# cruzryan/OpenDOG

Hardware: NVIDIA B200
Metric: env-steps/sec (device-timed) at 1/2/4/8 B200 vs ref mj_step on host cores (higher is better)
Workload: dtype f32

## Files before the change

### opendog_b200/csrc/odg_core.cuh

```cuda
#pragma once

#include <stdint.h>
#include <math.h>
#include <string.h>

#ifdef ODG_HOST_EMU
#define ODG_DEV inline
#define ODG_NOINLINE inline
#define ODG_RESTRICT
struct float4 { float x, y, z, w; };
float odg_emu_shfl_xor(float v, int m);
double odg_emu_shfl_xor_d(double v, int m);
static inline float odg_rsqrt(float x) { return 1.0f / sqrtf(x); }
static inline float odg_fmul_rn(float a, float b) { volatile float r = a * b; return r; }
static inline float odg_fadd_rn(float a, float b) { volatile float r = a + b; return r; }
static inline float odg_fsub_rn(float a, float b) { volatile float r = a - b; return r; }
static inline float odg_fdiv_rn(float a, float b) { volatile float r = a / b; return r; }
static inline float odg_fdiv_fast(float a, float b) { return a / b; }
static inline float odg_fma_rn(float a, float b, float c) { return fmaf(a, b, c); }
#ifdef ODG_EMU_STATS
void odg_emu_stat(int it, float rel_step, float alpha, int ls_passes, int nc_leg, float d10);
#endif
#define ODG_UNROLL
#define ODG_NO_UNROLL
// ... 93 lines not shown
  const float* mean;
  float* actions;
  float* cost;
};

struct StepArgs {
  const float* action;
  float* obs;
  float* reward;
  unsigned char* terminated; unsigned char* truncated;
  int mode;
  int want_info;
  float* x_position; float* y_position; float* distance; float* paw_forces; float* patterns_matches;
  float* lin_vel_reward; float* reward_ctrl; float* terminal_obs; unsigned char* paws_in_ground;
  int* gait_reward; float* qacc; int* ncon; float* fn_sum; int* solver_iters; int* ls_evals;
  float* reward_raw;
  float* cfrc_ext;
  float* task_terms;
};

struct V3 { float x, y, z; };
ODG_DEV V3 mk3(float x, float y, float z) { V3 r; r.x = x; r.y = y; r.z = z; return r; }
ODG_DEV V3 operator+(V3 a, V3 b) { return mk3(a.x + b.x, a.y + b.y, a.z + b.z); }
ODG_DEV V3 operator-(V3 a, V3 b) { return mk3(a.x - b.x, a.y - b.y, a.z - b.z); }
ODG_DEV V3 operator*(float s, V3 a) { return mk3(s * a.x, s * a.y, s * a.z); }
ODG_DEV V3 operator-(V3 a) { return mk3(-a.x, -a.y, -a.z); }
ODG_DEV float dot3(float ax, float ay, float az, float bx, float by, float bz) {
  return odg_fma_rn(az, bz, odg_fma_rn(ay, by, odg_fmul_rn(ax, bx)));
}
ODG_DEV float dot(V3 a, V3 b) { return dot3(a.x, a.y, a.z, b.x, b.y, b.z); }
ODG_DEV float cross1(float a, float b, float c, float d) { return odg_fma_rn(a, b, -odg_fmul_rn(c, d)); }
ODG_DEV V3 cross(V3 a, V3 b) { return mk3(cross1(a.y, b.z, a.z, b.y), cross1(a.z, b.x, a.x, b.z), cross1(a.x, b.y, a.y, b.x)); }
ODG_DEV float dot_acc(float acc, V3 a, V3 b) { return odg_fma_rn(a.z, b.z, odg_fma_rn(a.y, b.y, odg_fma_rn(a.x, b.x, acc))); }
ODG_DEV float cross1_acc(float acc, float a, float b, float c, float d) { return odg_fma_rn(a, b, odg_fma_rn(-c, d, acc)); }
ODG_DEV V3 cross_acc(V3 acc, V3 a, V3 b) {
  return mk3(cross1_acc(acc.x, a.y, b.z, a.z, b.y), cross1_acc(acc.y, a.z, b.x, a.x, b.z), cross1_acc(acc.z, a.x, b.y, a.y, b.x));
}
ODG_DEV float comp(V3 a, int i) { return i == 0 ? a.x : (i == 1 ? a.y : a.z); }

ODG_DEV float4 mk4(V3 v, float w) { float4 r; r.x = v.x; r.y = v.y; r.z = v.z; r.w = w; return r; }
ODG_DEV V3 xyz(float4 q) { return mk3(q.x, q.y, q.z); }
#ifdef ODG_HOST_EMU
static inline float odg_int_bits(int i) { float f; memcpy(&f, &i, 4); return f; }
static inline int odg_float_bits(float f) { int i; memcpy(&i, &f, 4); return i; }
#else
#define odg_int_bits __int_as_float
#define odg_float_bits __float_as_int
#endif

struct M3 { float m[9]; };
ODG_DEV V3 mul(const M3& R, V3 v) {
  return mk3(dot3(R.m[0], R.m[1], R.m[2], v.x, v.y, v.z), dot3(R.m[3], R.m[4], R.m[5], v.x, v.y, v.z),
             dot3(R.m[6], R.m[7], R.m[8], v.x, v.y, v.z));
}
ODG_DEV V3 tmul(const M3& R, V3 v) {
  return mk3(dot3(R.m[0], R.m[3], R.m[6], v.x, v.y, v.z), dot3(R.m[1], R.m[4], R.m[7], v.x, v.y, v.z),
             dot3(R.m[2], R.m[5], R.m[8], v.x, v.y, v.z));
}
ODG_DEV M3 mul(const M3& A, const M3& B) {
  M3 C;
  ODG_UNROLL for (int i = 0; i < 3; i++)
    ODG_UNROLL for (int j = 0; j < 3; j++)
      C.m[i * 3 + j] = A.m[i * 3] * B.m[j] + A.m[i * 3 + 1] * B.m[3 + j] + A.m[i * 3 + 2] * B.m[6 + j];
  return C;
}
ODG_DEV V3 col(const M3& R, int k) { return mk3(R.m[k], R.m[3 + k], R.m[6 + k]); }

struct S3 { float xx, xy, xz, yy, yz, zz; };
ODG_DEV V3 mul(const S3& A, V3 v) {
  return mk3(dot3(A.xx, A.xy, A.xz, v.x, v.y, v.z), dot3(A.xy, A.yy, A.yz, v.x, v.y, v.z),
             dot3(A.xz, A.yz, A.zz, v.x, v.y, v.z));
}
ODG_DEV S3 zero_s3() { S3 s; s.xx = s.xy = s.xz = s.yy = s.yz = s.zz = 0.f; return s; }
ODG_DEV void add_outer(S3& A, V3 a, V3 b) {
  A.xx += a.x * b.x; A.xy += a.x * b.y; A.xz += a.x * b.z; A.yy += a.y * b.y; A.yz += a.y * b.z; A.zz += a.z * b.z;
}
ODG_DEV S3 rotate_sym(const M3& R, const S3& A) {
  V3 c0 = mul(A, mk3(R.m[0], R.m[1], R.m[2]));
  V3 c1 = mul(A, mk3(R.m[3], R.m[4], R.m[5]));
  V3 c2 = mul(A, mk3(R.m[6], R.m[7], R.m[8]));
  V3 r0 = mk3(R.m[0], R.m[1], R.m[2]), r1 = mk3(R.m[3], R.m[4], R.m[5]), r2 = mk3(R.m[6], R.m[7], R.m[8]);
  S3 o;
  o.xx = dot(r0, c0); o.xy = dot(r0, c1); o.xz = dot(r0, c2);
  o.yy = dot(r1, c1); o.yz = dot(r1, c2); o.zz = dot(r2, c2);
  return o;
}

struct SpI { float m; V3 h; S3 I; };
ODG_DEV SpI spi_make(float mass, V3 c, const S3& Iw) {
  SpI s; s.m = mass; s.h = mass * c;
  float cc = dot(c, c);
  s.I.xx = Iw.xx + mass * (cc - c.x * c.x); s.I.yy = Iw.yy + mass * (cc - c.y * c.y); s.I.zz = Iw.zz + mass * (cc - c.z * c.z);
  s.I.xy = Iw.xy - mass * c.x * c.y; s.I.xz = Iw.xz - mass * c.x * c.z; s.I.yz = Iw.yz - mass * c.y * c.z;
  return s;
}
ODG_DEV SpI spi_add(const SpI& a, const SpI& b) {
  SpI s; s.m = a.m + b.m; s.h = a.h + b.h;
  s.I.xx = a.I.xx + b.I.xx; s.I.xy = a.I.xy + b.I.xy; s.I.xz = a.I.xz + b.I.xz;
  s.I.yy = a.I.yy + b.I.yy; s.I.yz = a.I.yz + b.I.yz; s.I.zz = a.I.zz + b.I.zz;
  return s;
}

#ifdef ODG_HOST_EMU
ODG_DEV float grp_xor(float v, int m, unsigned) { return odg_emu_shfl_xor(v, m); }
#else
ODG_DEV float grp_xor(float v, int m, unsigned gmask) { return __shfl_xor_sync(gmask, v, m); }
#endif
#ifdef ODG_HOST_EMU
ODG_DEV double grp_xor_d(double v, int m, unsigned) { return odg_emu_shfl_xor_d(v, m); }
#else
ODG_DEV double grp_xor_d(double v, int m, unsigned gmask) { return __shfl_xor_sync(gmask, v, m); }
#endif
#ifdef ODG_HOST_EMU
ODG_DEV void grp_sync(unsigned) { (void)odg_emu_shfl_xor(0.f, 1); }
#else
ODG_DEV void grp_sync(unsigned gmask) { __syncwarp(gmask); }
#endif
ODG_DEV float grp_sum(float v, unsigned gm) { v += grp_xor(v, 1, gm); v += grp_xor(v, 2, gm); return v; }
ODG_DEV float grp_sum21(float v, unsigned gm) { v += grp_xor(v, 2, gm); v += grp_xor(v, 1, gm); return v; }
constexpr int kRedVals = 28, kRedStride = 36, kRedGroup = 4 * kRedStride;
constexpr int kSupportCells = 24;
ODG_DEV void grp_sum28(float (&v)[kRedVals], float* ODG_RESTRICT s_red, int leg, unsigned gm) {
  grp_sync(gm);
  float4* mine = reinterpret_cast<float4*>(s_red + leg * kRedStride);
  ODG_UNROLL for (int k = 0; k < kRedVals / 4; k++) { float4 t; t.x = v[4 * k]; t.y = v[4 * k + 1]; t.z = v[4 * k + 2]; t.w = v[4 * k + 3]; mine[k] = t; }
  grp_sync(gm);
  float4* res = reinterpret_cast<float4*>(s_red);
  ODG_UNROLL for (int h = 0; h < 2; h++) {
    const int k = 2 * leg + h;
    const float4 a = reinterpret_cast<const float4*>(s_red)[k];
    const float4 b = reinterpret_cast<const float4*>(s_red + kRedStride)[k];
    const float4 c = reinterpret_cast<const float4*>(s_red + 2 * kRedStride)[k];
    const float4 d = reinterpret_cast<const float4*>(s_red + 3 * kRedStride)[k];
    float4 t;
    t.x = ((a.x + b.x) + c.x) + d.x; t.y = ((a.y + b.y) + c.y) + d.y; t.z = ((a.z + b.z) + c.z) + d.z; t.w = ((a.w + b.w) + c.w) + d.w;
    res[k] = t;
  }
  grp_sync(gm);
  ODG_UNROLL for (int k = 0; k < kRedVals / 4; k++) {
    const float4 t = res[k];
    v[4 * k] = t.x; v[4 * k + 1] = t.y; v[4 * k + 2] = t.z; v[4 * k + 3] = t.w;
  }
}
ODG_DEV void grp_sum_max2(float& sum, float& m0, float& m1, float* ODG_RESTRICT s_red, int leg, unsigned gm) {
  grp_sync(gm);
  float4 t; t.x = sum; t.y = m0; t.z = m1; t.w = 0.f;
  *reinterpret_cast<float4*>(s_red + leg * kRedStride) = t;
  grp_sync(gm);
  const float4 a = *reinterpret_cast<const float4*>(s_red), b = *reinterpret_cast<const float4*>(s_red + kRedStride);
  const float4 c = *reinterpret_cast<const float4*>(s_red + 2 * kRedStride), d = *reinterpret_cast<const float4*>(s_red + 3 * kRedStride);
  sum = ((a.x + b.x) + c.x) + d.x;
  m0 = fmaxf(fmaxf(a.y, b.y), fmaxf(c.y, d.y));
  m1 = fmaxf(fmaxf(a.z, b.z), fmaxf(c.z, d.z));
}
ODG_DEV float grp_max(float v, unsigned gm) { v = fmaxf(v, grp_xor(v, 1, gm)); v = fmaxf(v, grp_xor(v, 2, gm)); return v; }
ODG_DEV V3 grp_sum(V3 v, unsigned gm) { return mk3(grp_sum(v.x, gm), grp_sum(v.y, gm), grp_sum(v.z, gm)); }
ODG_DEV float grp_bcast(float v, int src_leg, int leg, unsigned gm) {
  float a = grp_xor(v, 1, gm); float m1 = ((leg ^ src_leg) & 1) ? a : v;
  float b = grp_xor(m1, 2, gm); return ((leg ^ src_leg) & 2) ? b : m1;
}

ODG_DEV void philox4x32(uint32_t k0, uint32_t k1, uint32_t c0, uint32_t c1, uint32_t c2, uint32_t c3, uint32_t out[4]) {
  ODG_UNROLL for (int r = 0; r < 10; r++) {
    uint64_t p0 = (uint64_t)0xD2511F53u * c0, p1 = (uint64_t)0xCD9E8D57u * c2;
    uint32_t n0 = (uint32_t)(p1 >> 32) ^ c1 ^ k0, n1 = (uint32_t)p1;
    uint32_t n2 = (uint32_t)(p0 >> 32) ^ c3 ^ k1, n3 = (uint32_t)p0;
    c0 = n0; c1 = n1; c2 = n2; c3 = n3; k0 += 0x9E3779B9u; k1 += 0xBB67AE85u;
  }
  out[0] = c0; out[1] = c1; out[2] = c2; out[3] = c3;
}
ODG_DEV float u01(uint32_t x) { return (float)(x >> 8) * 5.9604644775390625e-08f; }
constexpr uint32_t kStreamReset = 0x52534554u, kStreamDesvel = 0x44564c00u;

constexpr uint32_t kStreamMppi = 0x4d505049u;
#ifndef ODG_HOST_EMU
ODG_DEV void mppi_sample_row(const float* ODG_RESTRICT mean, float sigma, int n, int A, uint32_t seed_lo, uint32_t seed_hi,
                             uint32_t iteration, uint32_t t, float* ODG_RESTRICT action) {
  for (int blk = 0; blk * 4 < A; blk++) {
    uint32_t r[4];
    philox4x32(seed_lo, seed_hi, (uint32_t)n, iteration, (t << 8) | (uint32_t)blk, kStreamMppi, r);
    for (int pr = 0; pr < 2; pr++) {
      const float u1 = ((float)(r[2 * pr] >> 8) + 1.0f) * 5.9604644775390625e-08f;
      const float u2 = u01(r[2 * pr + 1]);
      const float rad = sqrtf(-2.0f * logf(u1));
      float sn, cs; sincosf(6.283185307179586f * u2, &sn, &cs);
      const float e[2] = { rad * cs, rad * sn };
      for (int q = 0; q < 2; q++) {
        const int a = blk * 4 + pr * 2 + q;
        if (a < A) action[(size_t)n * A + a] = fminf(1.f, fmaxf(-1.f, mean[a] + sigma * e[q]));
      }
    }
  }
}
#endif

ODG_NOINLINE float impedance_pow(float x, float mid, float power) {
  return x <= mid ? powf(x, power) / powf(mid, power - 1.f) : 1.f - powf(1.f - x, power) / powf(1.f - mid, power - 1.f);
}
ODG_DEV float impedance(const float* imp5, float pos_minus_margin) {
  const float d0 = imp5[0], d1 = imp5[1], width = imp5[2], mid = imp5[3], power = imp5[4];
  const bool flat = d0 == d1 || width <= 1e-15f;
  const float x = fminf(fabsf(odg_fdiv_fast(pos_minus_margin, flat ? 1.f : width)), 1.f);
  float y;
  if (power == 2.f) {
    const bool low = x <= mid;
    const float t = low ? x : 1.f - x;
    const float q = odg_fdiv_fast(t * t, low ? mid : 1.f - mid);
    y = low ? q : 1.f - q;
  } else if (power == 1.f) {
    y = x;
  } else {
    y = (x <= 0.f) ? 0.f : ((x >= 1.f) ? 1.f : impedance_pow(x, mid, power));
  }
  return flat ? 0.5f * (d0 + d1) : d0 + y * (d1 - d0);
}

ODG_DEV void fl_eval(float z, float f, float R, float D, float& g, float& hh) {
  g = fminf(fmaxf(D * z, -f), f);
  hh = fabsf(z) < R * f ? D : 0.f;
}

ODG_DEV int cone_eval(V3 z, float Dn, float Dt, float mu, float fri, float dmk, int condim, V3& g, S3& H) {
  if (condim == 1) { fri = 0.f; Dt = 0.f; }
  const float U1 = z.x * fri, U2 = z.y * fri, N = z.z * mu;
  const float T2 = odg_fma_rn(U1, U1, odg_fmul_rn(U2, U2));
  const float iT = odg_rsqrt(fmaxf(T2, 1e-20f));
  const float T = T2 * iT;
  const bool top = N >= mu * T;
  const bool bot = !top && (mu * N + T <= 0.f);
  const bool mid = !top && !bot;
  const float Dm = Dn * dmk;
  const float e = N - mu * T;
  const float ux = U1 * iT, uy = U2 * iT;
  const V3 w = mk3(-mu * ux * fri, -mu * uy * fri, mu);
  const float De = Dm * e;
  const float kap = -Dm * mu * e * iT;
  const float vx = -uy * fri, vy = ux * fri;
  g.x = mid ? De * w.x : (bot ? Dt * z.x : 0.f);
  g.y = mid ? De * w.y : (bot ? Dt * z.y : 0.f);
  g.z = mid ? De * w.z : (bot ? Dn * z.z : 0.f);
  const float Dwx = Dm * w.x, Dwy = Dm * w.y, kvx = kap * vx;
  H.xx = mid ? odg_fma_rn(Dwx, w.x, odg_fmul_rn(kvx, vx)) : (bot ? Dt : 0.f);
  H.yy = mid ? odg_fma_rn(Dwy, w.y, odg_fmul_rn(odg_fmul_rn(kap, vy), vy)) : (bot ? Dt : 0.f);
  H.zz = mid ? Dm * w.z * w.z : (bot ? Dn : 0.f);
  H.xy = mid ? odg_fma_rn(Dwx, w.y, odg_fmul_rn(kvx, vy)) : 0.f;
  H.xz = mid ? Dm * w.x * w.z : 0.f;
  H.yz = mid ? Dm * w.y * w.z : 0.f;
  return top ? 0 : (bot ? 1 : 2);
}

struct LineCoef { float N0, Nd, cA, cB, cC, q1, q2, Dm, mu; };
ODG_DEV LineCoef cone_line_prep(V3 z0, V3 dz, float Dn, float Dt, float mu, float fri, float dmk, int condim) {
  if (condim == 1) { fri = 0.f; Dt = 0.f; }
  const float U0x = odg_fmul_rn(z0.x, fri), U0y = odg_fmul_rn(z0.y, fri), Vx = odg_fmul_rn(dz.x, fri), Vy = odg_fmul_rn(dz.y, fri);
  LineCoef k;
  k.N0 = odg_fmul_rn(z0.z, mu); k.Nd = odg_fmul_rn(dz.z, mu);
  k.Dm = odg_fmul_rn(Dn, dmk); k.mu = mu;
  const float zt = odg_fma_rn(z0.x, dz.x, odg_fmul_rn(z0.y, dz.y)), dt = odg_fma_rn(dz.x, dz.x, odg_fmul_rn(dz.y, dz.y));
  k.q1 = odg_fma_rn(Dt, zt, odg_fmul_rn(odg_fmul_rn(Dn, z0.z), dz.z));
  k.q2 = odg_fma_rn(Dt, dt, odg_fmul_rn(odg_fmul_rn(Dn, dz.z), dz.z));
  k.cA = odg_fma_rn(U0x, U0x, odg_fmul_rn(U0y, U0y)); k.cB = odg_fma_rn(U0x, Vx, odg_fmul_rn(U0y, Vy));
  k.cC = odg_fma_rn(Vx, Vx, odg_fmul_rn(Vy, Vy));
  return k;
}
template <int W>
ODG_DEV void cone_line_eval(const LineCoef& c, const float (&al)[W], float (&f)[W]) {
  ODG_UNROLL for (int k = 0; k < W; k++) {
    const float a = al[k];
    const float N = c.N0 + a * c.Nd;
    const float UV = c.cB + a * c.cC;
    const float T2 = fmaxf(c.cA + a * (c.cB + UV), 0.f);
    const float iT = odg_rsqrt(fmaxf(T2, 1e-20f));
    const float T = T2 * iT;
    const float Td = UV * iT;
    const float e = N - c.mu * T;
    const float fmid = c.Dm * e * (c.Nd - c.mu * Td);
    const float fbot = c.q1 + a * c.q2;
    const bool bot = c.mu * N + T <= 0.f;
    f[k] += e >= 0.f ? 0.f : (bot ? fbot : fmid);
  }
}

struct Cone6 { float sc[6], D[6]; float mu, Dm; };
ODG_DEV Cone6 cone6_make(float Dn, float impratio, float mu, float fri, float dmk, float frt, float frr, float rt, float rr,
                         int condim = 3) {
  Cone6 k;
  if (condim == 1) { fri = 0.f; impratio = 0.f; }
  k.sc[0] = fri; k.sc[1] = fri; k.sc[2] = mu; k.sc[3] = frr; k.sc[4] = frr; k.sc[5] = frt;
  const float Dt = Dn * impratio;
  k.D[0] = Dt; k.D[1] = Dt; k.D[2] = Dn; k.D[3] = Dn * rr; k.D[4] = Dn * rr; k.D[5] = Dn * rt;
  k.mu = mu; k.Dm = Dn * dmk;
  return k;
}
ODG_DEV void cone6_eval(const float (&z)[6], const Cone6& k, float (&g)[6], float (&H)[6][6]) {
  float U[6];
  ODG_UNROLL for (int i = 0; i < 6; i++) U[i] = z[i] * k.sc[i];
  const float N = U[2], mu = k.mu;
  const float T2 = U[0] * U[0] + U[1] * U[1] + U[3] * U[3] + U[4] * U[4] + U[5] * U[5];
  const float iT = odg_rsqrt(fmaxf(T2, 1e-20f));
  const float T = T2 * iT;
  const bool top = N >= mu * T;
  const bool bot = !top && (mu * N + T <= 0.f);
  const bool mid = !top && !bot;
  const float e = N - mu * T;
  const float De = k.Dm * e, kap = -k.Dm * mu * e * iT;
  float u[6], w[6];
// ... 505 lines not shown
        const float4 q = FAT ? c_cj[c][j] : mk4(((j <= link) ? cross(ax[j], r - anc[j]) : mk3(0.f, 0.f, 0.f)), 0.f);
        cj[j] = xyz(q); cjw[j] = q.w;
        ap = ap + a_l[j] * cj[j];
      }
      V3 z = ap - xyz(af);
      c_z0[c] = mk4(z, 0.f);
      const float Dn = ra.w;
      if constexpr (kG) {
        V3 aj[NJL];
        V3 alb = a_b.w;
        ODG_UNROLL for (int j = 0; j < NJL; j++) {
          aj[j] = (j <= link) ? ax[j] : mk3(0.f, 0.f, 0.f);
          alb = alb + a_l[j] * aj[j];
        }
        const V3 za = alb - xyz(c_arefa[c]);
        c_z0a[c] = mk4(za, 0.f);
        const Cone6 K6 = cone6_make(Dn, C.impratio, C.slot_mu[s], C.slot_fri[s], C.slot_dmk[s], C.slot_frt[s], C.slot_frr[s],
                                    C.slot_dt_tor[s], C.slot_dt_roll[s], C.slot_condim[s]);
        const float z6[6] = { z.x, z.y, z.z, za.x, za.y, za.z };
        float g6[6], H6[6][6];
        cone6_eval(z6, K6, g6, H6);
        const V3 gL = mk3(g6[0], g6[1], g6[2]), gA = mk3(g6[3], g6[4], g6[5]);
        gb.t = gb.t + gL; gb.w = gb.w + cross(r, gL) + gA;
        auto HLL = [&](V3 v) { return mk3(H6[0][0] * v.x + H6[0][1] * v.y + H6[0][2] * v.z, H6[1][0] * v.x + H6[1][1] * v.y + H6[1][2] * v.z,
                                          H6[2][0] * v.x + H6[2][1] * v.y + H6[2][2] * v.z); };
        auto HLA = [&](V3 v) { return mk3(H6[0][3] * v.x + H6[0][4] * v.y + H6[0][5] * v.z, H6[1][3] * v.x + H6[1][4] * v.y + H6[1][5] * v.z,
                                          H6[2][3] * v.x + H6[2][4] * v.y + H6[2][5] * v.z); };
        auto HAL = [&](V3 v) { return mk3(H6[3][0] * v.x + H6[3][1] * v.y + H6[3][2] * v.z, H6[4][0] * v.x + H6[4][1] * v.y + H6[4][2] * v.z,
                                          H6[5][0] * v.x + H6[5][1] * v.y + H6[5][2] * v.z); };
        auto HAA = [&](V3 v) { return mk3(H6[3][3] * v.x + H6[3][4] * v.y + H6[3][5] * v.z, H6[4][3] * v.x + H6[4][4] * v.y + H6[4][5] * v.z,
                                          H6[5][3] * v.x + H6[5][4] * v.y + H6[5][5] * v.z); };
        Htt.xx += H6[0][0]; Htt.xy += H6[0][1]; Htt.xz += H6[0][2]; Htt.yy += H6[1][1]; Htt.yz += H6[1][2]; Htt.zz += H6[2][2];
        const V3 Xk[3] = { mk3(0.f, -r.z, r.y), mk3(r.z, 0.f, -r.x), mk3(-r.y, r.x, 0.f) };
        const V3 Ek[3] = { mk3(1.f, 0.f, 0.f), mk3(0.f, 1.f, 0.f), mk3(0.f, 0.f, 1.f) };
        V3 hL[3], hA[3];
        ODG_UNROLL for (int k = 0; k < 3; k++) { hL[k] = HLL(Xk[k]) + HLA(Ek[k]); hA[k] = HAL(Xk[k]) + HAA(Ek[k]); }
        ODG_UNROLL for (int k = 0; k < 3; k++) { Htw[0][k] += hL[k].x; Htw[1][k] += hL[k].y; Htw[2][k] += hL[k].z; }
        Hww.xx += dot(Xk[0], hL[0]) + hA[0].x; Hww.xy += dot(Xk[0], hL[1]) + hA[1].x; Hww.xz += dot(Xk[0], hL[2]) + hA[2].x;
        Hww.yy += dot(Xk[1], hL[1]) + hA[1].y; Hww.yz += dot(Xk[1], hL[2]) + hA[2].y; Hww.zz += dot(Xk[2], hL[2]) + hA[2].z;
        ODG_UNROLL for (int j = 0; j < NJL; j++) {
          const V3 hcL = HLL(cj[j]) + HLA(aj[j]), hcA = HAL(cj[j]) + HAA(aj[j]);
          g_l[j] += dot(cj[j], gL) + dot(aj[j], gA);
          Hlb[j].t = Hlb[j].t + hcL; Hlb[j].w = Hlb[j].w + cross(r, hcL) + hcA;
          ODG_UNROLL for (int i = 0; i <= j; i++) {
            float v = dot(cj[i], hcL) + dot(aj[i], hcA);
            Hll[j][i] += v; if (i != j) Hll[i][j] += v;
          }
        }
        continue;
      }
      V3 g; S3 H;
      if constexpr (kStash) cone_eval(z, Dn, cjw[1] != 0.f ? Dn * C.impratio : 0.f, cjw[0], cjw[1], af.w, 3, g, H);
      else cone_eval(z, Dn, Dn * C.impratio, C.slot_mu[s], C.slot_fri[s], C.slot_dmk[s], C.slot_condim[s], g, H);
      gb.t = gb.t + g; gb.w = cross_acc(gb.w, r, g);
      const V3 HX0 = mk3(cross1(H.xz, r.y, H.xy, r.z), cross1(H.yz, r.y, H.yy, r.z), cross1(H.zz, r.y, H.yz, r.z));
      const V3 HX1 = mk3(cross1(H.xx, r.z, H.xz, r.x), cross1(H.xy, r.z, H.yz, r.x), cross1(H.xz, r.z, H.zz, r.x));
      const V3 HX2 = mk3(cross1(H.xy, r.x, H.xx, r.y), cross1(H.yy, r.x, H.xy, r.y), cross1(H.yz, r.x, H.xz, r.y));
      Htt.xx += H.xx; Htt.xy += H.xy; Htt.xz += H.xz; Htt.yy += H.yy; Htt.yz += H.yz; Htt.zz += H.zz;
      Htw[0][0] += HX0.x; Htw[1][0] += HX0.y; Htw[2][0] += HX0.z;
      Htw[0][1] += HX1.x; Htw[1][1] += HX1.y; Htw[2][1] += HX1.z;
      Htw[0][2] += HX2.x; Htw[1][2] += HX2.y; Htw[2][2] += HX2.z;
      Hww.xx = cross1_acc(Hww.xx, r.y, HX0.z, r.z, HX0.y); Hww.xy = cross1_acc(Hww.xy, r.y, HX1.z, r.z, HX1.y);
      Hww.xz = cross1_acc(Hww.xz, r.y, HX2.z, r.z, HX2.y); Hww.yy = cross1_acc(Hww.yy, r.z, HX1.x, r.x, HX1.z);
      Hww.yz = cross1_acc(Hww.yz, r.z, HX2.x, r.x, HX2.z); Hww.zz = cross1_acc(Hww.zz, r.x, HX2.y, r.y, HX2.x);
      ODG_UNROLL for (int j = 0; j < NJL; j++) {
        V3 hc = mul(H, cj[j]);
        g_l[j] = dot_acc(g_l[j], cj[j], g);
        Hlb[j].t = Hlb[j].t + hc; Hlb[j].w = cross_acc(Hlb[j].w, r, hc);
        ODG_UNROLL for (int i = 0; i <= j; i++) Hll[j][i] = dot_acc(Hll[j][i], cj[i], hc);
      }
    }
    float iL[NJL];
    chol_small<NJL>(Hll, iL);
    Vec6 W[NJL]; float y[NJL];
    ODG_UNROLL for (int j = 0; j < NJL; j++) {
      W[j] = Hlb[j]; y[j] = g_l[j];
      ODG_UNROLL for (int i = 0; i < j; i++) {
        W[j].t = W[j].t - Hll[j][i] * W[i].t; W[j].w = W[j].w - Hll[j][i] * W[i].w;
        y[j] -= Hll[j][i] * y[i];
      }
      W[j].t = iL[j] * W[j].t; W[j].w = iL[j] * W[j].w; y[j] *= iL[j];
    }
    float S[6][6]; float rhs[6];
    {
      float P[6][6];
      ODG_UNROLL for (int i = 0; i < 6; i++) ODG_UNROLL for (int k = 0; k < 6; k++) P[i][k] = 0.f;
      P[0][0] = Htt.xx; P[1][0] = Htt.xy; P[2][0] = Htt.xz; P[1][1] = Htt.yy; P[2][1] = Htt.yz; P[2][2] = Htt.zz;
      P[3][3] = Hww.xx; P[4][3] = Hww.xy; P[5][3] = Hww.xz; P[4][4] = Hww.yy; P[5][4] = Hww.yz; P[5][5] = Hww.zz;
      ODG_UNROLL for (int i = 0; i < 3; i++) ODG_UNROLL for (int k = 0; k < 3; k++) P[3 + k][i] = Htw[i][k];
      P[0][0] += l0f * (T.m + C.base_arm_t[0]); P[1][1] += l0f * (T.m + C.base_arm_t[1]); P[2][2] += l0f * (T.m + C.base_arm_t[2]);
      P[3][3] += l0f * (T.I.xx + C.base_arm_r); P[4][3] += l0f * T.I.xy; P[5][3] += l0f * T.I.xz;
      P[4][4] += l0f * (T.I.yy + C.base_arm_r); P[5][4] += l0f * T.I.yz; P[5][5] += l0f * (T.I.zz + C.base_arm_r);
      P[3][1] += l0f * (-T.h.z); P[3][2] += l0f * (T.h.y);
      P[4][0] += l0f * (T.h.z);  P[4][2] += l0f * (-T.h.x);
      P[5][0] += l0f * (-T.h.y); P[5][1] += l0f * (T.h.x);
      float gbv[6] = { gb.t.x, gb.t.y, gb.t.z, gb.w.x, gb.w.y, gb.w.z };
      ODG_UNROLL for (int j = 0; j < NJL; j++) {
        float wl[6] = { W[j].t.x, W[j].t.y, W[j].t.z, W[j].w.x, W[j].w.y, W[j].w.z };
        ODG_UNROLL for (int i = 0; i < 6; i++) {
          ODG_UNROLL for (int k = 0; k <= i; k++) P[i][k] -= wl[i] * wl[k];
          gbv[i] -= wl[i] * y[j];
        }
      }
      float red[kRedVals];
      {
        int n = 0;
        ODG_UNROLL for (int i = 0; i < 6; i++) ODG_UNROLL for (int k = 0; k <= i; k++) red[n++] = P[i][k];
        ODG_UNROLL for (int i = 0; i < 6; i++) red[21 + i] = gbv[i];
        red[27] = 0.f;
      }
      grp_sum28(red, s_red, leg, gm);
      {
        int n = 0;
        ODG_UNROLL for (int i = 0; i < 6; i++) ODG_UNROLL for (int k = 0; k <= i; k++) S[i][k] = red[n++];
        ODG_UNROLL for (int i = 0; i < 6; i++) rhs[i] = -red[21 + i];
      }
    }
    chol6_solve(S, rhs);
    Vec6 p_b; p_b.t = mk3(rhs[0], rhs[1], rhs[2]); p_b.w = mk3(rhs[3], rhs[4], rhs[5]);
    float p_l[NJL];
    ODG_UNROLL for (int j = NJL - 1; j >= 0; j--) {
      float u = -y[j] - dot6(W[j], p_b);
      ODG_UNROLL for (int i = j + 1; i < NJL; i++) u -= Hll[i][j] * p_l[i];
      p_l[j] = u * iL[j];
    }
    float G = dot6(gauss_b, p_b), Hq = 0.f;
    {
      Vec6 Mpb = Mbb_mul(p_b);
      Hq = l0f * dot6(Mpb, p_b);
      ODG_UNROLL for (int j = 0; j < NJL; j++) {
        float mlp = dot6(Mlb[j], p_b);
        G += p_l[j] * gauss_l[j];
        float s = 2.f * mlp;
        ODG_UNROLL for (int i = 0; i < NJL; i++) s += Mll[j][i] * p_l[i];
        Hq += p_l[j] * s;
      }
    }
    auto line_coef = [&](int c, V3 dz, V3 dza) {
      const int s = kStash ? 0 : odg_float_bits(c_af[c].w);
      const float Dn = c_ra[c].w;
      if constexpr (kG) {
        const Cone6 K6 = cone6_make(Dn, C.impratio, C.slot_mu[s], C.slot_fri[s], C.slot_dmk[s], C.slot_frt[s], C.slot_frr[s],
                                    C.slot_dt_tor[s], C.slot_dt_roll[s], C.slot_condim[s]);
        const V3 zl = xyz(c_z0[c]), za = xyz(c_z0a[c]);
        const float z6[6] = { zl.x, zl.y, zl.z, za.x, za.y, za.z }, d6[6] = { dz.x, dz.y, dz.z, dza.x, dza.y, dza.z };
        return cone6_line_prep(z6, d6, K6);
      } else if constexpr (kStash) {
        const float mu = c_cj[c][0].w, fri = c_cj[c][1].w;
        return cone_line_prep(xyz(c_z0[c]), dz, Dn, fri != 0.f ? Dn * C.impratio : 0.f, mu, fri, c_af[c].w, 3);
      } else {
        return cone_line_prep(xyz(c_z0[c]), dz, Dn, Dn * C.impratio, C.slot_mu[s], C.slot_fri[s], C.slot_dmk[s], C.slot_condim[s]);
      }
    };
    ODG_NO_UNROLL for (int c = 0; c < nc; c++) {
      const int link = kStash ? 0 : C.slot_link[odg_float_bits(c_af[c].w)];
      const V3 r = xyz(c_ra[c]);
      V3 dz = cross_acc(p_b.t, p_b.w, r);
      ODG_UNROLL for (int j = 0; j < NJL; j++)
        dz = dz + p_l[j] * (FAT ? xyz(c_cj[c][j]) : ((j <= link) ? cross(ax[j], r - anc[j]) : mk3(0.f, 0.f, 0.f)));
      V3 dza = p_b.w;
      if constexpr (kG) {
        ODG_UNROLL for (int j = 0; j < NJL; j++) {
          const float on = fminf(fmaxf((float)(link - j + 1), 0.f), 1.f);
          dza = dza + (on * p_l[j]) * ax[j];
        }
      }
      if constexpr (FAT) {
        const LineCoef k = line_coef(c, dz, dza);
        float4 q;
        q.x = k.N0; q.y = k.Nd; q.z = k.cA; q.w = k.cB; c_lc[c][0] = q;
        q.x = k.cC; q.y = k.q1; q.z = k.q2; q.w = k.Dm; c_lc[c][1] = q;
        q.x = k.mu; q.y = 0.f; q.z = 0.f; q.w = 0.f; c_lc[c][2] = q;
      } else { c_dz[c] = mk4(dz, 0.f); if constexpr (kG) c_dza[c] = mk4(dza, 0.f); }
    }
    const float bf_zt = dot(bf_e, a_b.t) - bf_aref_t, bf_dzt = dot(bf_e, p_b.t);
    const float bf_zr = dot(bf_c, a_b.w) - bf_aref_r, bf_dzr = dot(bf_c, p_b.w);
    float d10 = dot6(gb, p_b);
    ODG_UNROLL for (int j = 0; j < NJL; j++) d10 += p_l[j] * g_l[j];
    float amax = 0.f, smax = 0.f;
    smax = fmaxf(fmaxf(fabsf(p_b.t.x), fabsf(p_b.t.y)), fmaxf(fabsf(p_b.t.z), fmaxf(fabsf(p_b.w.x), fmaxf(fabsf(p_b.w.y), fabsf(p_b.w.z)))));
    amax = fmaxf(fmaxf(fabsf(a_b.t.x), fabsf(a_b.t.y)), fmaxf(fabsf(a_b.t.z), fmaxf(fabsf(a_b.w.x), fmaxf(fabsf(a_b.w.y), fabsf(a_b.w.z)))));
    ODG_UNROLL for (int j = 0; j < NJL; j++) { smax = fmaxf(smax, fabsf(p_l[j])); amax = fmaxf(amax, fabsf(a_l[j])); }
    grp_sum_max2(d10, smax, amax, s_red, leg, gm);
    constexpr int LW = ODG_LS_WIDTH;
    auto evalw = [&](const float (&al)[LW], float (&f)[LW]) {
      ODG_UNROLL for (int k = 0; k < LW; k++) f[k] = G + al[k] * Hq;
      ODG_UNROLL for (int j = 0; j < NJL; j++) {
        const float fl = LCF(LC_FL, j);
        {
          const float D = LCF(LC_DFL, j), z0 = a_l[j] - aref_fl[j], dz = p_l[j];
          ODG_UNROLL for (int k = 0; k < LW; k++) f[k] += fminf(fmaxf(D * (z0 + al[k] * dz), -fl), fl) * dz;
        }
        {
          const float dzl = lim_sgn[j] * p_l[j], z0 = lim_sgn[j] * a_l[j] - lim_aref[j], Dd = lim_D[j] * dzl;
          ODG_UNROLL for (int k = 0; k < LW; k++) f[k] += fminf(z0 + al[k] * dzl, 0.f) * Dd;
        }
      }
      ODG_UNROLL for (int k = 0; k < LW; k++) f[k] += fminf(fmaxf(bf_Dt * (bf_zt + al[k] * bf_dzt), -bf_ft), bf_ft) * bf_dzt;
      ODG_UNROLL for (int k = 0; k < LW; k++) f[k] += fminf(fmaxf(bf_Dr * (bf_zr + al[k] * bf_dzr), -bf_fr), bf_fr) * bf_dzr;
      ODG_NO_UNROLL for (int c = 0; c < nc; c++) {
        if constexpr (FAT) {
          const float4 q0 = c_lc[c][0], q1 = c_lc[c][1], q2 = c_lc[c][2];
          LineCoef k;
          k.N0 = q0.x; k.Nd = q0.y; k.cA = q0.z; k.cB = q0.w; k.cC = q1.x; k.q1 = q1.y; k.q2 = q1.z; k.Dm = q1.w; k.mu = q2.x;
          cone_line_eval<LW>(k, al, f);
        } else {
          cone_line_eval<LW>(line_coef(c, xyz(c_dz[c]), kG ? xyz(c_dza[c]) : mk3(0.f, 0.f, 0.f)), al, f);
        }
      }
      ODG_UNROLL for (int k = 0; k < LW; k++) f[k] = grp_sum(f[k], gm);
    };
    auto eval4 = [&](const float (&al)[4], float (&f)[4]) {
      if (LW == 4) {
        float a4[LW], f4[LW];
        ODG_UNROLL for (int k = 0; k < LW; k++) a4[k] = al[k % 4];
        evalw(a4, f4);
        ODG_UNROLL for (int k = 0; k < LW; k++) f[k % 4] = f4[k];
      } else {
        ODG_NO_UNROLL for (int h = 0; h < 4 / LW; h++) {
          float aw[LW], fw[LW];
          ODG_UNROLL for (int k = 0; k < LW; k++) {
            aw[k] = al[k];
            ODG_UNROLL for (int g = 1; g < 4 / LW; g++) aw[k] = (h == g) ? al[(g * LW + k) % 4] : aw[k];
          }
          evalw(aw, fw);
          ODG_UNROLL for (int k = 0; k < LW; k++)
            ODG_UNROLL for (int g = 0; g < 4 / LW; g++) if (h == g) f[(g * LW + k) % 4] = fw[k];
        }
      }
    };
    const bool tiny = smax <= C.tol * (1.f + amax);
    float alpha = (tiny && d10 < 0.f) ? 1.f : 0.f;
#ifdef ODG_EMU_STATS
    const int ls_before = ls_evals;
#endif
    if (d10 < 0.f && !tiny) {
      const float ftol = C.ls_tol * fabsf(d10);
      float al[4] = { 0.25f, 0.5f, 1.f, 2.f }, f[4];
      float lo = 0.f, flo = d10, hi = -1.f, fhi = 0.f;
      bool done = false;
      ODG_NO_UNROLL for (int ls = 0; ls < C.ls_iters && !done; ls++) {
        {
          const bool first = ls == 0, ladder = lo == 0.f;
          const float w = (hi - lo) * 0.2f, lo0 = lo;
          const float lad[4] = { 0.008f, 0.04f, 0.2f, 0.6f };
          ODG_UNROLL for (int k = 0; k < 4; k++) {
            const float nxt = ladder ? lad[k] * hi : lo0 + w * (float)(k + 1);
            al[k] = first ? al[k] : nxt;
          }
        }
        eval4(al, f);
        ls_evals++;
        bool found = false;
        ODG_UNROLL for (int k = 0; k < 4; k++) {
          const bool hit = !done && fabsf(f[k]) <= ftol;
          alpha = hit ? al[k] : alpha; done = done || hit;
          const bool up = !found && f[k] >= 0.f, dn = !found && !(f[k] >= 0.f);
          hi = up ? al[k] : hi; fhi = up ? f[k] : fhi;
          lo = dn ? al[k] : lo; flo = dn ? f[k] : flo;
          found = found || up;
        }
        {
          const bool run = !done && hi < 0.f;
          alpha = run ? al[3] : alpha; done = done || run;
        }
      }
      if (!done) {
        alpha = lo - flo * odg_fdiv_fast(hi - lo, fhi - flo);
        alpha = (alpha >= lo && alpha <= hi) ? alpha : 0.5f * (lo + hi);
        alpha = (fhi < -0.1f * flo) ? hi : alpha;
      }
    }
#ifdef ODG_EMU_STATS
    if (lane0) odg_emu_stat(it, odg_fdiv_fast(smax, 1.f + amax), alpha, ls_evals - ls_before, nc, d10);
#endif
    a_b.t = a_b.t + alpha * p_b.t; a_b.w = a_b.w + alpha * p_b.w;
    ODG_UNROLL for (int j = 0; j < NJL; j++) a_l[j] += alpha * p_l[j];
    conv = tiny || !(d10 < 0.f);
  }
  work += iters + ls_evals;
  if (last) {
    out.a_b = a_b; ODG_UNROLL for (int j = 0; j < NJL; j++) out.a_l[j] = a_l[j];
    out.ncon = nc; out.iters = iters; out.ls_evals = ls_evals; out.R_last = R[NJL - 1];
    out.foot_contact = foot_last >= 0 ? 1 : 0;
    out.foot_force = mk3(0.f, 0.f, 0.f);
    if constexpr (kG) { ODG_UNROLL for (int q = 0; q <= NJL; q++) ODG_UNROLL for (int k = 0; k < 6; k++) out.cfrc[q][k] = 0.f; }
    float fn = 0.f;
    for (int c = 0; c < nc; c++) {
      const int s = kStash ? 0 : odg_float_bits(c_af[c].w);
      const int link = C.slot_link[s];
      const float Dn = c_ra[c].w;
      if (Dn == 0.f) continue;
      const V3 r = xyz(c_ra[c]);
      V3 ap = a_b.t + cross(a_b.w, r);
      ODG_UNROLL for (int j = 0; j < NJL; j++)
        ap = ap + a_l[j] * (FAT ? xyz(c_cj[c][j]) : ((j <= link) ? cross(ax[j], r - anc[j]) : mk3(0.f, 0.f, 0.f)));
      V3 g; S3 H;
      if constexpr (kG) {
        V3 alb = a_b.w;
        ODG_UNROLL for (int j = 0; j < NJL; j++) if (j <= link) alb = alb + a_l[j] * ax[j];
        const V3 zl = ap - xyz(c_af[c]), za = alb - xyz(c_arefa[c]);
        const Cone6 K6 = cone6_make(Dn, C.impratio, C.slot_mu[s], C.slot_fri[s], C.slot_dmk[s], C.slot_frt[s], C.slot_frr[s],
                                    C.slot_dt_tor[s], C.slot_dt_roll[s], C.slot_condim[s]);
        const float z6[6] = { zl.x, zl.y, zl.z, za.x, za.y, za.z };
        float g6[6], H6[6][6];
        cone6_eval(z6, K6, g6, H6);
        g = mk3(g6[0], g6[1], g6[2]);
        const V3 fw = -g, tw = mk3(-g6[3], -g6[4], -g6[5]);
        const V3 arm = r - odg_fdiv_rn(1.f, T.m) * T.h;
        const V3 tq = tw + cross(arm, fw);
        const int b = link < 0 ? NJL : link;
        ODG_UNROLL for (int q = 0; q <= NJL; q++) if (q == b) {
          out.cfrc[q][0] += tq.x; out.cfrc[q][1] += tq.y; out.cfrc[q][2] += tq.z;
          out.cfrc[q][3] += fw.x; out.cfrc[q][4] += fw.y; out.cfrc[q][5] += fw.z;
        }
      } else {
        if constexpr (kStash) {
          const float mu = c_cj[c][0].w, fri = c_cj[c][1].w;
          cone_eval(ap - xyz(c_af[c]), Dn, fri != 0.f ? Dn * C.impratio : 0.f, mu, fri, c_af[c].w, 3, g, H);
        } else {
          cone_eval(ap - xyz(c_af[c]), Dn, Dn * C.impratio, C.slot_mu[s], C.slot_fri[s], C.slot_dmk[s], C.slot_condim[s], g, H);
        }
      }
      fn += -g.z;
      if (c == foot_last) out.foot_force = mk3(-g.z, -g.y, g.x);
    }
    out.fn = fn;
  }
  const V3 acc_wl = tmul(R0, a_b.w);
  if (integrate) {
    const float h = C.h;
    Vec6 v_b = a_b; float v_l[NJL];
    ODG_UNROLL for (int j = 0; j < NJL; j++) v_l[j] = a_l[j];
    if (C.any_damping) {
      Vec6 rb = Mbb_mul(a_b);
      rb.t = l0f * rb.t; rb.w = l0f * rb.w;
      float rl[NJL], A[NJL][NJL];
      ODG_UNROLL for (int j = 0; j < NJL; j++) {
        float s = dot6(Mlb[j], a_b);
        ODG_UNROLL for (int i = 0; i < NJL; i++) { s += Mll[j][i] * a_l[i]; A[j][i] = Mll[j][i]; }
        A[j][j] += h * LCF(LC_DAMP, j);
        rl[j] = s;
        rb.t = rb.t + a_l[j] * Mlb[j].t; rb.w = rb.w + a_l[j] * Mlb[j].w;
      }
      spd_inverse<NJL>(A);
      Vec6 W[NJL]; float y[NJL];
      ODG_UNROLL for (int j = 0; j < NJL; j++) {
        W[j].t = mk3(0.f, 0.f, 0.f); W[j].w = mk3(0.f, 0.f, 0.f); y[j] = 0.f;
        ODG_UNROLL for (int i = 0; i < NJL; i++) {
          W[j].t = W[j].t + A[j][i] * Mlb[i].t; W[j].w = W[j].w + A[j][i] * Mlb[i].w;
          y[j] += A[j][i] * rl[i];
        }
      }
      float P[6][6], S[6][6], rhs[6];
      ODG_UNROLL for (int i = 0; i < 6; i++) ODG_UNROLL for (int k = 0; k < 6; k++) P[i][k] = 0.f;
      P[0][0] = l0f * (T.m + C.base_arm_t[0]); P[1][1] = l0f * (T.m + C.base_arm_t[1]); P[2][2] = l0f * (T.m + C.base_arm_t[2]);
      P[3][3] = l0f * (T.I.xx + C.base_arm_r); P[4][3] = l0f * T.I.xy; P[5][3] = l0f * T.I.xz;
      P[4][4] = l0f * (T.I.yy + C.base_arm_r); P[5][4] = l0f * T.I.yz; P[5][5] = l0f * (T.I.zz + C.base_arm_r);
      P[3][1] = l0f * (-T.h.z); P[3][2] = l0f * (T.h.y);
      P[4][0] = l0f * (T.h.z);  P[4][2] = l0f * (-T.h.x);
      P[5][0] = l0f * (-T.h.y); P[5][1] = l0f * (T.h.x);
      float rbv[6] = { rb.t.x, rb.t.y, rb.t.z, rb.w.x, rb.w.y, rb.w.z };
      ODG_UNROLL for (int j = 0; j < NJL; j++) {
        float hl[6] = { Mlb[j].t.x, Mlb[j].t.y, Mlb[j].t.z, Mlb[j].w.x, Mlb[j].w.y, Mlb[j].w.z };
        float wl[6] = { W[j].t.x, W[j].t.y, W[j].t.z, W[j].w.x, W[j].w.y, W[j].w.z };
        ODG_UNROLL for (int i = 0; i < 6; i++) {
          ODG_UNROLL for (int k = 0; k <= i; k++) P[i][k] -= hl[i] * wl[k];
          rbv[i] -= hl[i] * y[j];
        }
      }
      ODG_UNROLL for (int i = 0; i < 6; i++) {
        ODG_UNROLL for (int k = 0; k <= i; k++) S[i][k] = grp_sum(P[i][k], gm);
        rhs[i] = grp_sum(rbv[i], gm);
      }
      chol6_solve(S, rhs);
      v_b.t = mk3(rhs[0], rhs[1], rhs[2]); v_b.w = mk3(rhs[3], rhs[4], rhs[5]);
      ODG_UNROLL for (int j = 0; j < NJL; j++) v_l[j] = y[j] - dot6(W[j], v_b);
    }
    bv = bv + h * v_b.t;
    bwl = bwl + h * tmul(R0, v_b.w);
    ODG_UNROLL for (int j = 0; j < NJL; j++) { qd[j] += h * v_l[j]; q[j] += h * qd[j]; }
    bp = bp + h * bv;
    float wn = sqrtf(dot(bwl, bwl));
    if (wn > 1e-15f) {
      float s, c; sincosf(0.5f * h * wn, &s, &c);
      float k = s / wn;
      float dw = c, dx = k * bwl.x, dy = k * bwl.y, dz = k * bwl.z;
      float w = bq[0], x = bq[1], y = bq[2], z = bq[3];
      float nw = w * dw - x * dx - y * dy - z * dz;
      float nx = w * dx + x * dw + y * dz - z * dy;
      float ny = w * dy - x * dz + y * dw + z * dx;
      float nz = w * dz + x * dy - y * dx + z * dw;
      float in = odg_rsqrt(nw * nw + nx * nx + ny * ny + nz * nz);
      bq[0] = nw * in; bq[1] = nx * in; bq[2] = ny * in; bq[3] = nz * in;
    }
  }
  warm_v = a_b.t; warm_wl = acc_wl;
  ODG_UNROLL for (int j = 0; j < NJL; j++) warm_l[j] = a_l[j];
}

ODG_DEV void euler_from_quat(double w, double x, double y, double z, double& roll, double& pitch, double& yaw) {
  double t0 = 2.0 * (w * x + y * z), t1 = 1.0 - 2.0 * (x * x + y * y);
  roll = atan2(t0, t1);
  double t2 = 2.0 * (w * y - z * x);
  t2 = t2 > 1.0 ? 1.0 : t2; t2 = t2 < -1.0 ? -1.0 : t2;
  pitch = asin(t2);
  double t3 = 2.0 * (w * z + x * y), t4 = 1.0 - 2.0 * (y * y + z * z);
  yaw = atan2(t3, t4);
}

ODG_DEV void projected_gravity(const DevConst& C, const float (&quat)[4], float (&pg)[3]) {
  double e[3];
  euler_from_quat((double)quat[0], (double)quat[1], (double)quat[2], (double)quat[3], e[0], e[1], e[2]);
  const double d = (double)C.gx * e[0] + (double)C.gy * e[1] + (double)C.gz * e[2];
  const double v0 = d * e[0], v1 = d * e[1], v2 = d * e[2];
  const double n = sqrt(v0 * v0 + v1 * v1 + v2 * v2);
  pg[0] = (float)(n == 0.0 ? v0 : v0 / n); pg[1] = (float)(n == 0.0 ? v1 : v1 / n); pg[2] = (float)(n == 0.0 ? v2 : v2 / n);
}
// ... 369 lines not shown
```

Measured before the change: 10.00 million.

## Fuse contact line-coefficient prep with first line-search evaluation

Moves the per-contact dz/line-coefficient precompute loop inside the line-search branch and fuses it with the first 4-point evaluation, so each contact's coefficients are built and evaluated in a single pass. The first group reduction now goes through a single shared-memory float4 exchange instead of per-value shuffles, and the loop is restructured so later evaluations happen at the bottom. Precompute is skipped entirely when the line search is not needed (tiny step or non-descent direction). This may change register pressure, and in the non-FAT path c_dz is only written when the search runs.

```diff
diff --git a/opendog_b200/csrc/odg_core.cuh b/opendog_b200/csrc/odg_core.cuh
--- a/opendog_b200/csrc/odg_core.cuh
+++ b/opendog_b200/csrc/odg_core.cuh
@@ -269,6 +269,16 @@
   sum = ((a.x + b.x) + c.x) + d.x;
   m0 = fmaxf(fmaxf(a.y, b.y), fmaxf(c.y, d.y));
   m1 = fmaxf(fmaxf(a.z, b.z), fmaxf(c.z, d.z));
+}
+ODG_DEV void grp_sum4(float (&v)[4], float* ODG_RESTRICT s_red, int leg, unsigned gm) {
+  grp_sync(gm);
+  float4 t; t.x = v[0]; t.y = v[1]; t.z = v[2]; t.w = v[3];
+  *reinterpret_cast<float4*>(s_red + leg * kRedStride) = t;
+  grp_sync(gm);
+  const float4 a = *reinterpret_cast<const float4*>(s_red), b = *reinterpret_cast<const float4*>(s_red + kRedStride);
+  const float4 c = *reinterpret_cast<const float4*>(s_red + 2 * kRedStride), d = *reinterpret_cast<const float4*>(s_red + 3 * kRedStride);
+  v[0] = (a.x + b.x) + (c.x + d.x); v[1] = (a.y + b.y) + (c.y + d.y);
+  v[2] = (a.z + b.z) + (c.z + d.z); v[3] = (a.w + b.w) + (c.w + d.w);
 }
 ODG_DEV float grp_max(float v, unsigned gm) { v = fmaxf(v, grp_xor(v, 1, gm)); v = fmaxf(v, grp_xor(v, 2, gm)); return v; }
 ODG_DEV V3 grp_sum(V3 v, unsigned gm) { return mk3(grp_sum(v.x, gm), grp_sum(v.y, gm), grp_sum(v.z, gm)); }
@@ -1080,29 +1090,25 @@
         return cone_line_prep(xyz(c_z0[c]), dz, Dn, Dn * C.impratio, C.slot_mu[s], C.slot_fri[s], C.slot_dmk[s], C.slot_condim[s]);
       }
     };
-    ODG_NO_UNROLL for (int c = 0; c < nc; c++) {
-      const int link = kStash ? 0 : C.slot_link[odg_float_bits(c_af[c].w)];
-      const V3 r = xyz(c_ra[c]);
-      V3 dz = cross_acc(p_b.t, p_b.w, r);
-      ODG_UNROLL for (int j = 0; j < NJL; j++)
-        dz = dz + p_l[j] * (FAT ? xyz(c_cj[c][j]) : ((j <= link) ? cross(ax[j], r - anc[j]) : mk3(0.f, 0.f, 0.f)));
-      V3 dza = p_b.w;
-      if constexpr (kG) {
-        ODG_UNROLL for (int j = 0; j < NJL; j++) {
-          const float on = fminf(fmaxf((float)(link - j + 1), 0.f), 1.f);
-          dza = dza + (on * p_l[j]) * ax[j];
-        }
-      }
-      if constexpr (FAT) {
-        const LineCoef k = line_coef(c, dz, dza);
-        float4 q;
-        q.x = k.N0; q.y = k.Nd; q.z = k.cA; q.w = k.cB; c_lc[c][0] = q;
-        q.x = k.cC; q.y = k.q1; q.z = k.q2; q.w = k.Dm; c_lc[c][1] = q;
-        q.x = k.mu; q.y = 0.f; q.z = 0.f; q.w = 0.f; c_lc[c][2] = q;
-      } else { c_dz[c] = mk4(dz, 0.f); if constexpr (kG) c_dza[c] = mk4(dza, 0.f); }
-    }
     const float bf_zt = dot(bf_e, a_b.t) - bf_aref_t, bf_dzt = dot(bf_e, p_b.t);
     const float bf_zr = dot(bf_c, a_b.w) - bf_aref_r, bf_dzr = dot(bf_c, p_b.w);
+    auto rows_eval = [&](const auto& al, auto& f) {
+      constexpr int W = sizeof(al) / sizeof(al[0]);
+      ODG_UNROLL for (int k = 0; k < W; k++) f[k] = G + al[k] * Hq;
+      ODG_UNROLL for (int j = 0; j < NJL; j++) {
+        const float fl = LCF(LC_FL, j);
+        {
+          const float D = LCF(LC_DFL, j), z0 = a_l[j] - aref_fl[j], dz = p_l[j];
+          ODG_UNROLL for (int k = 0; k < W; k++) f[k] += fminf(fmaxf(D * (z0 + al[k] * dz), -fl), fl) * dz;
+        }
+        {
+          const float dzl = lim_sgn[j] * p_l[j], z0 = lim_sgn[j] * a_l[j] - lim_aref[j], Dd = lim_D[j] * dzl;
+          ODG_UNROLL for (int k = 0; k < W; k++) f[k] += fminf(z0 + al[k] * dzl, 0.f) * Dd;
+        }
+      }
+      ODG_UNROLL for (int k = 0; k < W; k++) f[k] += fminf(fmaxf(bf_Dt * (bf_zt + al[k] * bf_dzt), -bf_ft), bf_ft) * bf_dzt;
+      ODG_UNROLL for (int k = 0; k < W; k++) f[k] += fminf(fmaxf(bf_Dr * (bf_zr + al[k] * bf_dzr), -bf_fr), bf_fr) * bf_dzr;
+    };
     float d10 = dot6(gb, p_b);
     ODG_UNROLL for (int j = 0; j < NJL; j++) d10 += p_l[j] * g_l[j];
     float amax = 0.f, smax = 0.f;
@@ -1112,20 +1118,7 @@
     grp_sum_max2(d10, smax, amax, s_red, leg, gm);
     constexpr int LW = ODG_LS_WIDTH;
     auto evalw = [&](const float (&al)[LW], float (&f)[LW]) {
-      ODG_UNROLL for (int k = 0; k < LW; k++) f[k] = G + al[k] * Hq;
-      ODG_UNROLL for (int j = 0; j < NJL; j++) {
-        const float fl = LCF(LC_FL, j);
-        {
-          const float D = LCF(LC_DFL, j), z0 = a_l[j] - aref_fl[j], dz = p_l[j];
-          ODG_UNROLL for (int k = 0; k < LW; k++) f[k] += fminf(fmaxf(D * (z0 + al[k] * dz), -fl), fl) * dz;
-        }
-        {
-          const float dzl = lim_sgn[j] * p_l[j], z0 = lim_sgn[j] * a_l[j] - lim_aref[j], Dd = lim_D[j] * dzl;
-          ODG_UNROLL for (int k = 0; k < LW; k++) f[k] += fminf(z0 + al[k] * dzl, 0.f) * Dd;
-        }
-      }
-      ODG_UNROLL for (int k = 0; k < LW; k++) f[k] += fminf(fmaxf(bf_Dt * (bf_zt + al[k] * bf_dzt), -bf_ft), bf_ft) * bf_dzt;
-      ODG_UNROLL for (int k = 0; k < LW; k++) f[k] += fminf(fmaxf(bf_Dr * (bf_zr + al[k] * bf_dzr), -bf_fr), bf_fr) * bf_dzr;
+      rows_eval(al, f);
       ODG_NO_UNROLL for (int c = 0; c < nc; c++) {
         if constexpr (FAT) {
           const float4 q0 = c_lc[c][0], q1 = c_lc[c][1], q2 = c_lc[c][2];
@@ -1163,21 +1156,35 @@
     const int ls_before = ls_evals;
 #endif
     if (d10 < 0.f && !tiny) {
+      float al[4] = { 0.25f, 0.5f, 1.f, 2.f }, f[4];
+      rows_eval(al, f);
+      ODG_NO_UNROLL for (int c = 0; c < nc; c++) {
+        const int link = kStash ? 0 : C.slot_link[odg_float_bits(c_af[c].w)];
+        const V3 r = xyz(c_ra[c]);
+        V3 dz = cross_acc(p_b.t, p_b.w, r);
+        ODG_UNROLL for (int j = 0; j < NJL; j++)
+          dz = dz + p_l[j] * (FAT ? xyz(c_cj[c][j]) : ((j <= link) ? cross(ax[j], r - anc[j]) : mk3(0.f, 0.f, 0.f)));
+        V3 dza = p_b.w;
+        if constexpr (kG) {
+          ODG_UNROLL for (int j = 0; j < NJL; j++) {
+            const float on = fminf(fmaxf((float)(link - j + 1), 0.f), 1.f);
+            dza = dza + (on * p_l[j]) * ax[j];
+          }
+        }
+        const LineCoef k = line_coef(c, dz, dza);
+        cone_line_eval<4>(k, al, f);
+        if constexpr (FAT) {
+          float4 q;
+          q.x = k.N0; q.y = k.Nd; q.z = k.cA; q.w = k.cB; c_lc[c][0] = q;
+          q.x = k.cC; q.y = k.q1; q.z = k.q2; q.w = k.Dm; c_lc[c][1] = q;
+          q.x = k.mu; q.y = 0.f; q.z = 0.f; q.w = 0.f; c_lc[c][2] = q;
+        } else { c_dz[c] = mk4(dz, 0.f); if constexpr (kG) c_dza[c] = mk4(dza, 0.f); }
+      }
+      grp_sum4(f, s_red, leg, gm);
       const float ftol = C.ls_tol * fabsf(d10);
-      float al[4] = { 0.25f, 0.5f, 1.f, 2.f }, f[4];
       float lo = 0.f, flo = d10, hi = -1.f, fhi = 0.f;
       bool done = false;
-      ODG_NO_UNROLL for (int ls = 0; ls < C.ls_iters && !done; ls++) {
-        {
-          const bool first = ls == 0, ladder = lo == 0.f;
-          const float w = (hi - lo) * 0.2f, lo0 = lo;
-          const float lad[4] = { 0.008f, 0.04f, 0.2f, 0.6f };
-          ODG_UNROLL for (int k = 0; k < 4; k++) {
-            const float nxt = ladder ? lad[k] * hi : lo0 + w * (float)(k + 1);
-            al[k] = first ? al[k] : nxt;
-          }
-        }
-        eval4(al, f);
+      ODG_NO_UNROLL for (int ls = 1;; ls++) {
         ls_evals++;
         bool found = false;
         ODG_UNROLL for (int k = 0; k < 4; k++) {
@@ -1192,6 +1199,14 @@
           const bool run = !done && hi < 0.f;
           alpha = run ? al[3] : alpha; done = done || run;
         }
+        if (done || ls >= C.ls_iters) break;
+        {
+          const bool ladder = lo == 0.f;
+          const float w = (hi - lo) * 0.2f, lo0 = lo;
+          const float lad[4] = { 0.008f, 0.04f, 0.2f, 0.6f };
+          ODG_UNROLL for (int k = 0; k < 4; k++) al[k] = ladder ? lad[k] * hi : lo0 + w * (float)(k + 1);
+        }
+        eval4(al, f);
       }
       if (!done) {
         alpha = lo - flo * odg_fdiv_fast(hi - lo, fhi - flo);
```

Result: faster. 10.18 million (median of 6 runs) (+1.7%).
